# EBI-Metagenomics/deciphon-old

Measured on AMD Instinct MI355X. Metric: Gcell-updates/sec, higher is better.
Workload: dtype f32

## Files before the change

deciphon-old_amd/csrc/dcp_gpu.hip:

```cpp
#include "dcp_kernels.h"
#include "dcp_f64.h"

#include <hip/hip_runtime.h>

#include <algorithm>
#include <cmath>
#include <cstdarg>
#include <cstdio>
#include <cstring>
#include <limits>
#include <map>
#include <new>
#include <string>
#include <queue>
#include <vector>

namespace
{

struct SizeClass
{
    int R, W;
    unsigned cap() const { return 64u * (unsigned)R * (unsigned)W; }
};
// ... 1414 lines not shown
    {
        if (c->qorder_q0 != q_begin || c->qorder_q1 != q_end || c->qorder_nt != ql_nt)
        {
            unsigned const NTq = ql_nt, slots = NTq / 64u;
            std::vector<uint32_t> ord(nq);
            for (unsigned i = 0; i < nq; ++i)
                ord[i] = i;
            std::stable_sort(ord.begin(), ord.end(), [&](uint32_t x, uint32_t y) {
                return c->seq_len[q_begin + x] < c->seq_len[q_begin + y];
            });
            std::vector<unsigned> len_sorted(nq);
            for (unsigned i = 0; i < nq; ++i)
                len_sorted[i] = c->seq_len[q_begin + ord[i]];
            QlPlan const plan = plan_query_groups(len_sorted.data(), nq, slots);
            unsigned const nqb = plan.nqb;
            if ((uint64_t)plan.plane_rows * NTq * 4u > 0xffffffffull)
                return c->fail(DCP_ENOMEM, "sequences too long for the query-lane kernel (%u plane rows): use kernel = 1", plan.plane_rows);
            size_t const nslot_words = (size_t)nqb * slots + 1u, ngroup_words = plan.groups.size() * 4u;
            size_t const need_stage = (size_t)nq + nqb + 1u + nslot_words + ngroup_words;
            if (!c->ev_qstage) HIP_TRY(c, hipEventCreateWithFlags(&c->ev_qstage, hipEventDisableTiming));
            else HIP_TRY(c, hipEventSynchronize(c->ev_qstage));
            if (c->h_qstage_n < need_stage)
            {
                if (c->h_qstage) (void)hipHostFree(c->h_qstage);
                c->h_qstage = nullptr, c->h_qstage_n = 0;
                HIP_TRY(c, hipHostMalloc((void **)&c->h_qstage, need_stage * sizeof(uint32_t), hipHostMallocDefault));
                c->h_qstage_n = need_stage;
            }
            uint32_t *const h_ord = c->h_qstage, *const wt_off = h_ord + nq, *const h_slots = wt_off + nqb + 1u,
                           *const h_groups = h_slots + nslot_words;
            static_assert(sizeof(dcp_ql_group) == 4 * sizeof(uint32_t), "group records travel as four words");
// ... 85 lines not shown
                qa.redo_base[k] = (unsigned)tot;
                qa.redo_cap[k] = cap;
                tot += cap;
                uint64_t const tpb = dcp_rowsweep_tasks_per_block(kClasses[k].W);
                uint64_t g = std::min<uint64_t>((cap + tpb - 1) / tpb, 8ull * c->num_cus);
                redo_grid[k] = (unsigned)((g + 7) / 8 * 8);
            }
            if (c->d_redo.n < tot) HIP_TRY(c, c->d_redo.alloc((size_t)tot));
        }
        if (!c->d_redo_n.p) HIP_TRY(c, c->d_redo_n.alloc(DCP_MAX_CLASSES + 2));
        HIP_TRY(c, hipMemsetAsync(c->d_redo_n.p, 0, (DCP_MAX_CLASSES + 2) * sizeof(unsigned), c->stream));
        qa.redo = c->d_redo.p;
        qa.redo_n = c->d_redo_n.p;
        qa.redo_overflow = c->d_redo_n.p + DCP_MAX_CLASSES;
        qa.ring_error = c->d_redo_n.p + DCP_MAX_CLASSES + 1;
        uint64_t const per_block = (uint64_t)dcp_qlane_scratch_planes() * (uint64_t)qa.plane_rows * NT;
        uint64_t const budget = (uint64_t)64 << 28;
        uint64_t fit = per_block ? budget / per_block : 0;
        uint64_t const resident_blocks = (uint64_t)ql_blocks_per_cu * c->num_cus;
        unsigned nblocks = (unsigned)std::min<uint64_t>(std::min<uint64_t>(ntasks, resident_blocks), fit);
        if (use_w3) nblocks = (nblocks + 2u) / 3u * 3u;
        if (nblocks == 0)
            return c->fail(DCP_ENOMEM, "sequences too long for the query-lane kernel (%u plane rows): use kernel = 1", qa.plane_rows);
        size_t const need = (size_t)nblocks * per_block;
        if (c->d_scratch.n < need) HIP_TRY(c, c->d_scratch.alloc(need));
        qa.scratch = c->d_scratch.p;
        HIP_TRY(c, hipMemsetAsync(c->d_task_counter.p, 0, sizeof(unsigned), c->stream));
        HIP_TRY(c, hipEventRecord(c->ev_start, c->stream));
        if (two_stage ? dcp_launch_qlane2(&qa, nblocks, c->stream)
                      : use_w3 ? dcp_launch_qlane_w3(&qa, nblocks / 3u, c->stream)
                               : dcp_launch_qlane(&qa, nblocks, NT, c->stream))
// ... 611 lines not shown
```

deciphon-old_amd/csrc/dcp_kernels.h:

```cpp
#ifndef DCP_KERNELS_H
#define DCP_KERNELS_H

#include "dcp_host.h"
#include <stdint.h>

struct dcp_prof_meta
{
    uint64_t emis_off;
    uint32_t trans_off;
    uint32_t core_size;
    uint32_t ldk;
    uint32_t pidx;
    uint32_t flags;
    uint32_t width;
};
#define DCP_PROF_EXACT_E 1u

struct dcp_mp_group
{
    uint64_t emis_off;
    uint32_t trans_off;
    uint32_t ldk;
    uint32_t in_off;
    uint32_t nparts;
// ... 172 lines not shown
unsigned dcp_segsweep_blocks(unsigned nprof, unsigned nq);
int dcp_launch_rowsweep_grid(int R, int W, dcp_scan_args const *a, int stg, unsigned bw, void *stream,
                             unsigned pad_lds,
                             int prefetch2);
unsigned dcp_rowsweep_max_block_waves(int R, int W, int stg);
unsigned dcp_rowsweep_stage_bytes(int R, int stg);
int dcp_launch_qlane(dcp_qlane_args const *a, unsigned nblocks, unsigned nt, void *stream);
int dcp_launch_qlane2(dcp_qlane_args const *a, unsigned nblocks, void *stream);
unsigned dcp_qlane2_lds_bytes(void);
int dcp_launch_qlane_w3(dcp_qlane_args const *a, unsigned nblocks, void *stream);
int dcp_launch_qlane_transpose(dcp_qlane_args const *a, unsigned nt, void *stream);
void dcp_launch_trace(dcp_trace_args const *a, unsigned nhits, void *stream);
int dcp_launch_trace_forward(int R, int W, dcp_scan_args const *a, unsigned nblocks, void *stream);
unsigned dcp_qlane_block_size(void);
unsigned dcp_qlane_tile_nodes(void);
unsigned dcp_qlane_scratch_planes(void);
unsigned dcp_qlane_diag_build(void);
unsigned dcp_qlane_group_rows(unsigned lmax);
unsigned dcp_qlane_window_planes(void);
unsigned dcp_qlane_exact_e_by_redo(void);
#ifdef __cplusplus
}
#endif

#endif
```

deciphon-old_amd/csrc/dcp_qlane.hip:

```cpp
#include "dcp_kernels.h"

#include <hip/hip_runtime.h>
#include <type_traits>

namespace
{
constexpr int NC = DCP_NCODES;

#ifndef DCP_QLANE_RECOMPUTE_B
#define DCP_QLANE_RECOMPUTE_B 1
#endif
constexpr bool kRecomputeB = DCP_QLANE_RECOMPUTE_B != 0;
#ifndef DCP_QLANE_WD
#define DCP_QLANE_WD 5
#endif
constexpr unsigned kWD = DCP_QLANE_WD;
constexpr unsigned kPlanes = kRecomputeB ? 3u : 4u;
#ifndef DCP_QLANE_DIAG
#define DCP_QLANE_DIAG 0
#endif

#ifndef DCP_QL_WPLANE
#define DCP_QL_WPLANE 1
#endif
#ifndef DCP_QL_IN16
#define DCP_QL_IN16 1
#endif
#ifndef DCP_QL_EM
#define DCP_QL_EM 1
#endif
constexpr bool kWPlane = DCP_QL_WPLANE != 0, kIn16 = DCP_QL_IN16 != 0, kEM = DCP_QL_EM != 0;

// ... 88 lines not shown
        }
    }
}

__device__ __forceinline__ float ld_off(float const *base, unsigned boff)
{
    return *reinterpret_cast<float const *>(reinterpret_cast<char const *>(base) + boff);
}
typedef uint32_t const __attribute__((address_space(1))) *gu32_ptr;
typedef uint16_t const __attribute__((address_space(1))) *gu16_ptr;
typedef char const __attribute__((address_space(1))) *gchar_ptr;
__device__ __forceinline__ void st_off(float *base, unsigned boff, float v)
{
    *reinterpret_cast<float *>(reinterpret_cast<char *>(base) + boff) = v;
}

struct Ring
{
    float B[5], Xm[5], Xd[5], Em[5];
};

enum
{
    IO_HBM = 1,
    IO_LDS = 2
};
constexpr unsigned kRD = 16;
constexpr unsigned kRLanes = 256;
constexpr unsigned kRingPlaneBytes = kRD * kRLanes * 4u;
#ifndef DCP_Q2_SKEW
#define DCP_Q2_SKEW 4
#endif
#ifndef DCP_Q2_HYST
#define DCP_Q2_HYST 1
// ... 51 lines not shown
constexpr unsigned kRingSpinBound = 1u << 23;
constexpr unsigned kRingPoison = 0x7fffff00u;
__device__ __forceinline__ unsigned ring_wait(LdsLink const &lk, unsigned need)
{
    lds_uint *flag = (lds_uint *)(lk.base + lk.peer_flag);
    unsigned v = __builtin_amdgcn_readfirstlane(flag_load(flag));
#if DCP_Q2_BOUND
    unsigned spins = 0;
#pragma nounroll
    while (v < need)
    {
        __builtin_amdgcn_s_sleep(DCP_Q2_SLEEP);
        v = __builtin_amdgcn_readfirstlane(flag_load(flag));
        if (__builtin_expect(++spins == kRingSpinBound, 0))
        {
            typedef unsigned __attribute__((address_space(1))) *gerr_ptr;
            gerr_ptr const err = *(gerr_ptr __attribute__((address_space(3))) *)(lk.base + kL2Err);
            __hip_atomic_store(err, 1u, __ATOMIC_RELAXED, __HIP_MEMORY_SCOPE_AGENT);
            flag_store((lds_uint *)(lk.base + kL2Abort), 1u);
            flag_store(flag, kRingPoison);
            v = kRingPoison;
            __builtin_amdgcn_s_waitcnt(0x0070);
        }
    }
#else
    while (v < need)
    {
        __builtin_amdgcn_s_sleep(DCP_Q2_SLEEP);
        v = __builtin_amdgcn_readfirstlane(flag_load(flag));
    }
#endif
    DCP_ISA_MARK("DCP_RING_ACQUIRED");
    return v;
}
__device__ __forceinline__ float ring_ld(LdsLink const &lk, unsigned rowoff, unsigned plane)
{
    return *(lds_float *)(lk.base + ((rowoff & (kRingPlaneBytes - 1u)) | kL2Ring) + plane * kRingPlaneBytes);
}
__device__ __forceinline__ void ring_st(LdsLink const &lk, unsigned rowoff, unsigned plane, float v)
{
    *(lds_float *)(lk.base + ((rowoff & (kRingPlaneBytes - 1u)) | kL2Ring) + plane * kRingPlaneBytes) = v;
}
__device__ __forceinline__ void ring_publish(LdsLink const &lk, unsigned rowoff, unsigned row)
{
    flag_store((lds_uint *)(lk.base + lk.my_flag + (rowoff & (kRLanes * 4u - 1u))), row);
}

template <bool FIRST>
__device__ __forceinline__ void ring_fetch_x(Ring &r, int slot, float const *pXm, float const *pXd,
                                             float const *pEm, unsigned off)
{
    if constexpr (!FIRST)
    {
        r.Xm[slot] = ld_off(pXm, off);
        r.Xd[slot] = ld_off(pXd, off);
        r.Em[slot] = ld_off(pEm, off);
    }
}
template <bool FIRST>
__device__ __forceinline__ void ring_fetch_b(Ring &r, int slot, float const *pB, unsigned off)
{
    if constexpr (!kRecomputeB && !FIRST) r.B[slot] = ld_off(pB, off);
}
template <bool FIRST>
__device__ __forceinline__ void ring_fetch(Ring &r, int slot, float const *pB, float const *pXm,
                                           float const *pXd, float const *pEm, unsigned off)
{
    ring_fetch_x<FIRST>(r, slot, pXm, pXd, pEm, off);
    ring_fetch_b<FIRST>(r, slot, pB, off);
}

struct GatherOff
{
    unsigned a[5];
};
template <unsigned BASE> struct GatherMasks
{
    unsigned base, m[4];
    __device__ __forceinline__ GatherMasks()
    {
        static_assert((BASE & 0x3fffu) == 0u, "the base must not overlap the window's 14 bits");
        base = BASE;
        if constexpr (BASE != 0u) asm volatile("" : "+s"(base));
#pragma unroll
        for (int l = 0; l < 4; ++l)
// ... 31 lines not shown
            reinterpret_cast<char const *>(tabIN) + (IN16 ? g.a[l] + first[l] * 16u : (g.a[l] >> 1) + first[l] * 8u));
        in.eI[l] = v.x;
        in.eN[l] = v.y;
    }
}

template <int R> __device__ __forceinline__ float comp(float4 const &v)
{
    return R == 0 ? v.x : R == 1 ? v.y : R == 2 ? v.z : v.w;
}

template <int G, bool FIRST, bool LAST, int PH, int NT, int D, int IN = IO_HBM, int OUT = IO_HBM, unsigned TBASE = 0u,
          bool IN16 = kIn16>
__device__ __forceinline__ void ql_row(QState<G> &s, TileTrans<G> const &tr, float const *tabM,
                                       float2 const *tabIN, GatherOff &go,
                                       unsigned wn, RowIn &in, Ring &ring, float *pB, float *pXm,
                                       float *pXd, float *pEm, unsigned &off, LaneXt const &xt,
                                       bool live, bool at_end, bool &dirty, SweepOut &o,
                                       LdsLink const &lk, unsigned jrow, GatherMasks<TBASE> const &gm
#if DCP_QLANE_DIAG & 4
                                       , unsigned &off2, unsigned din
#endif
                                       )
{
    constexpr int KT = 4 * G;
    constexpr int s1 = (PH + 4) % 5, s2 = (PH + 3) % 5, s3 = (PH + 2) % 5, s4 = (PH + 1) % 5, s5 = PH;
    float const ni = ninf();

    static_assert(G <= 2, "gather_match<GROUP> is instantiated for groups 0 and 1");
    float4 e[G > 1 ? G - 1 : 1][5];
    if constexpr (G > 1)
    {
#pragma unroll
        for (int l = 0; l < 5; ++l)
            e[0][l] = gather_match<1>(tabM, go, l);
    }

    {
        constexpr int per_row = ((FIRST || IN != IO_HBM) ? 0 : 3) + ((LAST || OUT != IO_HBM) ? 0 : 3) +
                                ((!kRecomputeB && !FIRST) ? 1 : 0) + ((!kRecomputeB && FIRST) ? 1 : 0) + 1;
        constexpr int vm = ((D < (int)kWD ? D : (int)kWD) - 1) * per_row;
        constexpr int lgkm = G > 1 ? 5 : 0;
        __builtin_amdgcn_s_waitcnt((vm & 15) | ((vm >> 4) << 14) | (7 << 4) | (lgkm << 8));
    }
    __builtin_amdgcn_sched_barrier(0);
    float Xm = ni, Xd = ni, E = ni, Bj = ring.B[PH];
    if constexpr (!FIRST)
    {
        Xm = ring.Xm[PH];
        Xd = ring.Xd[PH];
        E = ring.Em[PH];
    }
    float eI[5], eN[5];
#pragma unroll
    for (int l = 0; l < 5; ++l)
    {
        eI[l] = in.eI[l];
        eN[l] = in.eN[l];
    }

    if constexpr (FIRST || kRecomputeB)
    {
        float const N = mx5(s.PN[s1] + eN[0], s.PN[s2] + eN[1], s.PN[s3] + eN[2],
                            s.PN[s4] + eN[3], s.PN[s5] + eN[4]);
        s.PN[PH] = N + xt.NN;
        Bj = N + xt.NB;
        if constexpr (FIRST)
        {
            float const Rn = mx5(s.PR[s1] + eN[0], s.PR[s2] + eN[1], s.PR[s3] + eN[2],
                                 s.PR[s4] + eN[3], s.PR[s5] + eN[4]);
            s.PR[PH] = Rn + xt.RR;
            o.Rn = at_end ? Rn : o.Rn;
            if constexpr (!kRecomputeB) st_off(pB, off, Bj);
        }
    }

    float pm = ni, pi = ni, pd = ni;
    float m_even = ni;
    auto node = [&](int k, float e0, float e1, float e2, float e3, float e4) {
        float const m = mx5(s.P[s1][k] + e0, s.P[s2][k] + e1, s.P[s3][k] + e2, s.P[s4][k] + e3,
                            s.P[s5][k] + e4);
        float const iv = mx5(s.Q[s1][k] + eI[0], s.Q[s2][k] + eI[1], s.Q[s3][k] + eI[2],
                             s.Q[s4][k] + eI[3], s.Q[s5][k] + eI[4]);
        float d, pin;
        if (k == 0)
        {
            d = Xd;
            pin = Xm;
// ... 11 lines not shown
        else E = mx3(E, m, d);
        s.P[PH][k] = fmaxf(Bj + tr.ent[k], pin);
        s.Q[PH][k] = fmaxf(m + tr.mi[k], iv + tr.ii[k]);
        pm = m, pi = iv, pd = d;
    };

    node(0, in.e0[0].x, in.e0[1].x, in.e0[2].x, in.e0[3].x, in.e0[4].x);
    node(1, in.e0[0].y, in.e0[1].y, in.e0[2].y, in.e0[3].y, in.e0[4].y);
    node(2, in.e0[0].z, in.e0[1].z, in.e0[2].z, in.e0[3].z, in.e0[4].z);
    node(3, in.e0[0].w, in.e0[1].w, in.e0[2].w, in.e0[3].w, in.e0[4].w);

    if constexpr (!FIRST && IN == IO_HBM)
    {
        asm volatile("" : "+v"(off) : "v"(E));
#if DCP_QLANE_DIAG & 4
        ring_fetch_x<FIRST>(ring, (PH + D) % 5, pXm + din, pXd + din, pEm + din, off);
#else
        ring_fetch_x<FIRST>(ring, (PH + D) % 5, pXm + D * NT, pXd + D * NT, pEm + D * NT, off);
#endif
    }

    __builtin_amdgcn_s_waitcnt(0xC07F | (0 << 8));
    go = gather_off<TBASE>(wn, gm);
    ql_fetch<G, FIRST, LAST, IN16>(in, tabM, tabIN, go);
    if constexpr (!FIRST && IN == IO_LDS)
    {
        constexpr int sl = (PH + 1) % 5;
        DCP_ISA_MARK("DCP_RING_TAKE");
        unsigned const nxt = off + kRLanes * 4u;
        ring.Xm[sl] = ring_ld(lk, nxt, 0);
        ring.Xd[sl] = ring_ld(lk, nxt, 1);
        ring.Em[sl] = ring_ld(lk, nxt, 2);
        DCP_ISA_MARK("DCP_RING_TAKEN");
        ring_publish(lk, off, jrow + 1u);
        DCP_ISA_MARK("DCP_RING_TAKE_END");
    }

#pragma unroll
    for (int g = 1; g < G; ++g)
    {
        float4 const *eg = e[g - 1];
        node(4 * g + 0, eg[0].x, eg[1].x, eg[2].x, eg[3].x, eg[4].x);
        node(4 * g + 1, eg[0].y, eg[1].y, eg[2].y, eg[3].y, eg[4].y);
        node(4 * g + 2, eg[0].z, eg[1].z, eg[2].z, eg[3].z, eg[4].z);
        node(4 * g + 3, eg[0].w, eg[1].w, eg[2].w, eg[3].w, eg[4].w);
    }

    if constexpr (!kRecomputeB && !FIRST)
    {
        asm volatile("" : "+v"(off) : "v"(pm));
        ring_fetch_b<FIRST>(ring, (PH + D) % 5, pB + D * NT, off);
    }

    if constexpr (!LAST)
    {
        float const oXm = mx3(pm + tr.mm[KT], pi + tr.im[KT], pd + tr.dm[KT]);
        float const oXd = fmaxf(pm + tr.md[KT], pd + tr.dd[KT]);
        if constexpr (OUT == IO_LDS)
        {
            DCP_ISA_MARK("DCP_RING_DATA");
            ring_st(lk, off, 0, oXm);
            ring_st(lk, off, 1, oXd);
            ring_st(lk, off, 2, E);
            DCP_ISA_MARK("DCP_RING_FLAG");
            ring_publish(lk, off, jrow);
            DCP_ISA_MARK("DCP_RING_DATA_END");
        }
        else
        {
#if DCP_QLANE_DIAG & 4
            unsigned const offw = off2;
#else
            unsigned const offw = off;
#endif
            st_off(pXm, offw, oXm);
            st_off(pXd, offw, oXd);
            st_off(pEm, offw, E);
        }
    }
    else
    {
        float const J = mx5(s.PJ[s1] + eN[0], s.PJ[s2] + eN[1], s.PJ[s3] + eN[2], s.PJ[s4] + eN[3],
                            s.PJ[s5] + eN[4]);
        float const C = mx5(s.PC[s1] + eN[0], s.PC[s2] + eN[1], s.PC[s3] + eN[2], s.PC[s4] + eN[3],
                            s.PC[s5] + eN[4]);
        float const B1 = fmaxf(E + xt.EB, J + xt.JB);
        dirty = dirty || (live && B1 > Bj);
        s.PJ[PH] = fmaxf(E + xt.EJ, J + xt.JJ);
        s.PC[PH] = fmaxf(E + xt.EC, C + xt.CC);
        o.E = at_end ? E : o.E;
        o.C = at_end ? C : o.C;
    }
}

template <int G, bool FIRST, bool LAST, int NT, int D, int IN = IO_HBM, int OUT = IO_HBM, unsigned TBASE = 0u,
          bool IN16 = kIn16>
__device__ __forceinline__ void ql_sweep(cfloat *tt, float const *tabM, float2 const *tabIN,
                                         uint32_t const *__restrict__ wordsT, unsigned rowbase,
                                         unsigned L, unsigned Lwave, bool active, float *sc,
                                         size_t plane, unsigned tid, LaneXt const &xt, bool &dirty,
                                         SweepOut &o, LdsLink lk
#if DCP_QLANE_DIAG & 4
                                         , unsigned tile_odd
#endif
                                         )
{
    constexpr int KT = 4 * G;
#if DCP_QLANE_DIAG & 4
    unsigned const rowstep = tile_odd ? 0u : (unsigned)NT;
    unsigned const rowstep_out = tile_odd ? (unsigned)NT : 0u;
    unsigned const din = (unsigned)D * rowstep;
    unsigned off2 = tid * 4u;
#else
    constexpr unsigned rowstep = (DCP_QLANE_DIAG & 2) ? 0u : (unsigned)NT;
#endif
// ... 5 lines not shown
    for (int h = 0; h < 5; ++h)
    {
#pragma unroll
        for (int k = 0; k < KT; ++k)
            s.P[h][k] = ni, s.Q[h][k] = ni;
        s.PN[h] = ni, s.PR[h] = ni, s.PJ[h] = ni, s.PC[h] = ni;
    }
    {
        float const B0 = 0.0f + xt.SB;
#pragma unroll
        for (int k = 0; k < KT; ++k)
            s.P[0][k] = B0 + tr.ent[k];
        s.PN[0] = 0.0f + xt.SN;
        s.PR[0] = 0.0f;
    }
    float *pXm = sc, *pXd = sc + plane, *pEm = sc + 2 * plane, *pB = sc + (kRecomputeB ? 0 : 3) * plane;
    unsigned off = (rowbase * (unsigned)NT + tid) * 4u;

    unsigned j = 1;
    static_assert(kWPlane, "the packed-word sequence planes are gone (round 4): a slot's groups are addressed by plane row");
    typedef uint16_t wq_t;
    wq_t wq[5];
    unsigned w;
    unsigned lane2 = tid * 2u;
    gu16_ptr const wpl = (gu16_ptr)wordsT + (size_t)rowbase * (unsigned)NT;
    asm volatile("" : "+v"(lane2));
    {
        w = wpl[NT + tid];
#pragma unroll
        for (int r = 2; r < 7; ++r)
            wq[r % 5] = wpl[r * NT + tid];
        __builtin_amdgcn_sched_barrier(0);
        __builtin_amdgcn_s_waitcnt(0x0F70);
    }
    RowIn in;
    Ring ring;
#pragma unroll
    for (int l = 0; l < 5; ++l)
    {
        in.e0[l] = float4{ni, ni, ni, ni}, in.eI[l] = ni, in.eN[l] = ni;
        ring.B[l] = ring.Xm[l] = ring.Xd[l] = ring.Em[l] = ni;
    }
    GatherMasks<TBASE> const gm;
    GatherOff go = gather_off<TBASE>(w, gm);
    ql_fetch<G, FIRST, LAST, IN16>(in, tabM, tabIN, go);
    if constexpr (!FIRST && IN == IO_LDS)
    {
        static_assert(NT == (int)kRLanes, "the ring's row stride is the scratch planes' row stride");
        unsigned const need0 = rowbase + (Lwave < kRingSkew ? Lwave : kRingSkew);
        lk.seen = ring_wait(lk, need0);
        DCP_ISA_MARK("DCP_RING_TAKE");
        ring.Xm[1] = ring_ld(lk, off, 0);
        ring.Xd[1] = ring_ld(lk, off, 1);
        ring.Em[1] = ring_ld(lk, off, 2);
        DCP_ISA_MARK("DCP_RING_TAKEN");
        ring_publish(lk, off, rowbase + 1u);
        DCP_ISA_MARK("DCP_RING_TAKE_END");
    }
    else
    {
        lk.seen = 0u;
#pragma unroll
        for (int r = 0; r < D; ++r)
            ring_fetch<(FIRST || IN != IO_HBM)>(ring, (r + 1) % 5, pB, pXm, pXd, pEm, off + (unsigned)r * rowstep * 4u);
    }

#if DCP_QLANE_DIAG & 8
#ifndef DCP_QLANE_DIAG_ROWS
#define DCP_QLANE_DIAG_ROWS 256u
#endif
#define QL_DIAG8_WRAP off &= (DCP_QLANE_DIAG_ROWS * (unsigned)NT * 4u - 1u);
#else
#define QL_DIAG8_WRAP
#endif
#if DCP_QLANE_DIAG & 4
#define QL_DIAG4_ARGS , off2, din
#define QL_DIAG4_STEP off2 += rowstep_out * 4u;
#else
#define QL_DIAG4_ARGS
#define QL_DIAG4_STEP
#endif
#define QL_ROW(PH)                                                                         \
    {                                                                                      \
                                                 \
        unsigned const pos = j + 1u;                                                       \
        ql_row<G, FIRST, LAST, PH, NT, D, IN, OUT, TBASE, IN16>(s, tr, tabM, tabIN, go,              \
                                   (unsigned)wq[(PH + 1) % 5], in, ring, pB, pXm,                    \
                                   pXd, pEm, off, xt, active && j <= L, active && j == L,  \
                                   dirty, o, lk, rowbase + j, gm QL_DIAG4_ARGS);           \
        {    \
             \
             \
             \
             \
            gu16_ptr wrow = wpl + (pos + 5u) * (unsigned)NT;                                     \
            asm volatile("" : "+s"(wrow));                                                   \
            asm volatile("" : "+v"(lane2));  \
            wq[(PH + 1) % 5] = *(gu16_ptr)((gchar_ptr)wrow + lane2);                          \
        }                                                                                    \
        off += rowstep * 4u;                                                                     \
        QL_DIAG8_WRAP                                                                            \
        QL_DIAG4_STEP                                                                            \
        ++j;                                                                               \
// ... 54 lines not shown
    g.rowbase = gd->rowbase;
    g.has = lane < nq;
    g.q = g.has ? a.qorder[qfirst + lane] : 0u;
    g.L = g.has ? a.seq_len[g.q] : 0u;
    g.Lwave = gd->lmax;
    float const *__restrict__ x = a.xtrans + (size_t)g.q * DCP_XSTRIDE;
    g.xt.RR = x[DCP_X_RR], g.xt.SB = x[DCP_X_SB], g.xt.SN = x[DCP_X_SN], g.xt.NN = x[DCP_X_NN];
    g.xt.NB = x[DCP_X_NB], g.xt.ET = x[DCP_X_ET], g.xt.EC = x[DCP_X_EC], g.xt.CC = x[DCP_X_CC];
    g.xt.CT = x[DCP_X_CT], g.xt.EB = x[DCP_X_EB], g.xt.EJ = x[DCP_X_EJ], g.xt.JJ = x[DCP_X_JJ];
    g.xt.JB = x[DCP_X_JB];
    __builtin_amdgcn_s_waitcnt(0x0F70);
    __builtin_amdgcn_sched_barrier(0);
}
__device__ __forceinline__ unsigned park_off(GroupLane const &g, unsigned NT, unsigned col)
{
    return ((g.rowbase + g.Lwave + 8u) * NT + col) * 4u;
}

__device__ __forceinline__ void ql_publish(dcp_qlane_args const &a, dcp_ql_prof const &pm, unsigned q, float nul, float alt,
                                           bool redo)
{
    if (redo)
    {
        unsigned const cls = pm.cls;
        unsigned const i = atomicAdd(a.redo_n + cls, 1u);
        if (i < a.redo_cap[cls]) a.redo[a.redo_base[cls] + i] = dcp_pair{q, pm.rs_slot};
        else *a.redo_overflow = 1u;
        return;
    }
    size_t const oi = (size_t)q * a.nprof_total + pm.pidx;
    if (a.out_null) a.out_null[oi] = nul;
// ... 6 lines not shown
    }
}

}

template <int G, int NT, int D, bool ROWS = false>
__global__ __launch_bounds__(NT, NT / 128) void viterbi_qlane_kernel(dcp_qlane_args a)
{
    constexpr int KT = 4 * G;
    constexpr int TAB_FLOATS = G * NC * 4;
    __shared__ __attribute__((aligned(16))) float lds[TAB_FLOATS + (kIn16 ? 4 : 2) * NC];
    __shared__ unsigned s_task;
    float *tabM = lds;
    float2 *tabIN = reinterpret_cast<float2 *>(lds + TAB_FLOATS);
    unsigned const tid = threadIdx.x;
    size_t const plane = (size_t)a.plane_rows * (unsigned)NT;
    float *const sc = a.scratch + (size_t)blockIdx.x * kPlanes * plane;
    constexpr unsigned SLOTS = (unsigned)NT / 64u;

    for (;;)
    {
        if (tid == 0) s_task = atomicAdd(a.task_counter, 1u);
        __syncthreads();
        unsigned const task = __builtin_amdgcn_readfirstlane(s_task);
        __syncthreads();
        if (task >= a.ntasks) break;
        unsigned const slot = a.nprof - 1u - task / a.nqblocks;
        unsigned const qb = task % a.nqblocks;
        dcp_ql_prof const pm = a.profs[slot];
        unsigned const T = pm.ntiles;
        unsigned const sidx = __builtin_amdgcn_readfirstlane(qb * SLOTS + (tid >> 6));
        cu32 *sf = (cu32 *)(unsigned long long)a.slot_first;
// ... 17 lines not shown
            cfloat *tt = as_const(a.ttrans + pm.ttrans_off + (size_t)t * (KT + 1) * 8);
            bool const first = t == 0, last = t + 1 == T;
            for (unsigned gi = g0; gi < g1; ++gi)
            {
                if (!(single && t_loaded)) load_group(a, gi, tid & 63u, g);
                t_loaded = true;
                if (g.Lwave == 0u) continue;
                SweepOut o{ninf(), ninf(), ninf()};
                bool dirty = false;
#if DCP_QLANE_DIAG & 4
#define QL_DIAG4_TILE , (t & 1u)
#else
#define QL_DIAG4_TILE
#endif
#define QL_SWEEP(F, L_)                                                                          \
    ql_sweep<G, F, L_, NT, D>(tt, tabM, tabIN, wordsT, g.rowbase, g.L, g.Lwave, g.has, sc, plane, tid, g.xt, dirty, o, LdsLink{} QL_DIAG4_TILE)
                if (first && last) QL_SWEEP(true, true);
                else if (first) QL_SWEEP(true, false);
                else if (last) QL_SWEEP(false, true);
                else QL_SWEEP(false, false);
#undef QL_SWEEP
                unsigned const po = park_off(g, (unsigned)NT, tid);
                if (first && !last) st_off(sc, po, o.Rn);
                if (last && g.has)
                {
                    float const nul = first ? o.Rn : ld_off(sc, po);
                    ql_publish(a, pm, g.q, nul, fmaxf(o.E + g.xt.ET, o.C + g.xt.CT), dirty || (kEM && pm.needs_exact_e));
                }
            }
        }
    }
// ... 3 lines not shown
__global__ __launch_bounds__(512, 2) void viterbi_qlane2_kernel(dcp_qlane_args a)
{
    constexpr int NT = (int)kRLanes;
    constexpr int KT = 4 * G;
    __shared__ __attribute__((aligned(16))) float lds[kL2Bytes / 4u];
    unsigned const wv = threadIdx.x >> 6;
#if DCP_Q2_STAGEMAP == 0
    unsigned const stage = __builtin_amdgcn_readfirstlane(wv & 1u);
    unsigned const tid = ((wv >> 1) << 6) | (threadIdx.x & 63u);
#else
    unsigned const stage = __builtin_amdgcn_readfirstlane(wv >> 2);
    unsigned const tid = threadIdx.x & 255u;
#endif
    unsigned *const s_task_p = reinterpret_cast<unsigned *>(lds + kL2Task / 4u);
    float *const tabM = lds + (stage ? kL2Tab1 / 4u : 0u);
    size_t const plane = (size_t)a.plane_rows * (unsigned)NT;
    float *const sc = a.scratch + (size_t)blockIdx.x * kPlanes * plane;
    constexpr unsigned SLOTS = (unsigned)NT / 64u;

#if DCP_Q2_PRIO == 1
    if (stage == 1u) __builtin_amdgcn_s_setprio(1);
#elif DCP_Q2_PRIO == 2
    if (stage == 0u) __builtin_amdgcn_s_setprio(1);
#endif
    LdsLink lk;
    lk.base = (lds_char *)lds;
    lk.my_flag = stage == 0u ? kL2FlagP : kL2FlagC;
    lk.peer_flag = (stage == 0u ? kL2FlagC : kL2FlagP) + (tid & ~63u) * 4u;
    lk.seen = 0u;
    if (threadIdx.x == 0) *(unsigned **)(lds + kL2Err / 4u) = a.ring_error;
    unsigned *const s_abort_p = reinterpret_cast<unsigned *>(lds + kL2Abort / 4u);

// ... 41 lines not shown
            if (!mine || (stalled && st == 0u) || __builtin_amdgcn_readfirstlane(*s_abort_p) != 0u) continue;
            cfloat *tt = as_const(a.ttrans + pm.ttrans_off + (size_t)t * (KT + 1) * 8);
            bool const first = t == 0u, last = t + 1u == T;
#if DCP_QLANE_DIAG & 4
#error "the two-stage kernel has no DIAG=4 build"
#endif
            for (unsigned gi = g0; gi < g1; ++gi)
            {
                if (!(single && t_loaded)) load_group(a, gi, tid & 63u, g);
                t_loaded = true;
                if (g.Lwave == 0u) continue;
                SweepOut o{ninf(), ninf(), ninf()};
                bool dirty = false;
#define QL2_SWEEP(F, L_, IN_, OUT_, TB_)                                                                  \
    ql_sweep<G, F, L_, NT, D, IN_, OUT_, TB_, false>(tt, lds, reinterpret_cast<float2 const *>(lds + (kL2TabIN - TB_ / 2u) / 4u), \
                                              wordsT, g.rowbase, g.L, g.Lwave, g.has, sc, plane, tid, g.xt, dirty, o, lk)
                if (stage == 0u)
                {
                    if (first && last) QL2_SWEEP(true, true, IO_HBM, IO_HBM, 0u);
                    else if (first) QL2_SWEEP(true, false, IO_HBM, IO_LDS, 0u);
                    else if (last) QL2_SWEEP(false, true, IO_HBM, IO_HBM, 0u);
                    else QL2_SWEEP(false, false, IO_HBM, IO_LDS, 0u);
                }
                else
                {
                    if (last) QL2_SWEEP(false, true, IO_LDS, IO_HBM, kL2Tab1);
                    else QL2_SWEEP(false, false, IO_LDS, IO_HBM, kL2Tab1);
                }
#undef QL2_SWEEP
                unsigned const po = park_off(g, (unsigned)NT, tid);
                if (first) st_off(sc, po, o.Rn);
                if (last)
                {
                    st_off(sc + plane, po, fmaxf(o.E + g.xt.ET, o.C + g.xt.CT));
                    st_off(sc + 2 * plane, po, dirty ? 1.0f : 0.0f);
                }
            }
        }
        __syncthreads();

        if (stage != final_stage) continue;
        for (unsigned gi = g0; gi < g1; ++gi)
        {
            cgroup *gd = (cgroup *)(unsigned long long)(a.groups + gi);
            GroupLane ge;
            ge.rowbase = gd->rowbase, ge.Lwave = gd->lmax;
            if (ge.Lwave == 0u || (tid & 63u) >= gd->nq) continue;
            unsigned const q = a.qorder[gd->qfirst + (tid & 63u)];
            unsigned const po = park_off(ge, (unsigned)NT, tid);
            float const nul = ld_off(sc, po), alt = ld_off(sc + plane, po);
            bool const dirty = ld_off(sc + 2 * plane, po) != 0.0f;
            ql_publish(a, pm, q, nul, alt, dirty || (kEM && pm.needs_exact_e));
        }
    }
}

template <int G, int D, bool ROWS = false>
__global__ __launch_bounds__(192, 1) void viterbi_qlane_w3_kernel(dcp_qlane_args a)
{
    constexpr int NT = 64;
    constexpr int KT = 4 * G;
    constexpr int TAB_FLOATS = G * NC * 4;
    constexpr int SLICE = TAB_FLOATS + 2 * NC;
    __shared__ __attribute__((aligned(16))) float lds[3 * SLICE];
    unsigned const wv = __builtin_amdgcn_readfirstlane(threadIdx.x >> 6);
    unsigned const tid = threadIdx.x & 63u;
    float *const tabM = lds + wv * SLICE;
    float2 *const tabIN = reinterpret_cast<float2 *>(tabM + TAB_FLOATS);
    size_t const plane = (size_t)a.plane_rows * (unsigned)NT;
    float *const sc = a.scratch + ((size_t)blockIdx.x * 3u + wv) * kPlanes * plane;

    for (;;)
    {
        unsigned t0 = 0;
        if (tid == 0) t0 = atomicAdd(a.task_counter, 1u);
        unsigned const task = __builtin_amdgcn_readfirstlane(t0);
        if (task >= a.ntasks) break;
        unsigned const slot = a.nprof - 1u - task / a.nqblocks;
        unsigned const qb = task % a.nqblocks;
        dcp_ql_prof const pm = a.profs[slot];
        unsigned const T = pm.ntiles;
        cu32 *sf = (cu32 *)(unsigned long long)a.slot_first;
        unsigned const g0 = sf[qb], g1 = sf[qb + 1u];
        uint32_t const *__restrict__ wordsT = a.words_t + __builtin_amdgcn_readfirstlane(a.wt_off[qb]);
        {
// ... 7 lines not shown
        bool t_loaded = false;
        for (unsigned t = 0; t < T; ++t)
        {
            stage_tile_image<G, ROWS>(tabM, a, pm, t, tid, (unsigned)NT);
            compiler_fence();
            cfloat *tt = as_const(a.ttrans + pm.ttrans_off + (size_t)t * (KT + 1) * 8);
            bool const first = t == 0, last = t + 1 == T;
            for (unsigned gi = g0; gi < g1; ++gi)
            {
                if (!(single && t_loaded)) load_group(a, gi, tid, g);
                t_loaded = true;
                if (g.Lwave == 0u) continue;
                SweepOut o{ninf(), ninf(), ninf()};
                bool dirty = false;
#define QLW_SWEEP(F, L_)                                                                                  \
    ql_sweep<G, F, L_, NT, D, IO_HBM, IO_HBM, 0u, false>(tt, tabM, tabIN, wordsT, g.rowbase, g.L, g.Lwave, g.has, sc, plane, tid, g.xt, dirty, o, LdsLink{})
                if (first && last) QLW_SWEEP(true, true);
                else if (first) QLW_SWEEP(true, false);
                else if (last) QLW_SWEEP(false, true);
                else QLW_SWEEP(false, false);
#undef QLW_SWEEP
                unsigned const po = park_off(g, (unsigned)NT, tid);
                if (first && !last) st_off(sc, po, o.Rn);
                if (last && g.has)
                {
                    float const nul = first ? o.Rn : ld_off(sc, po);
                    ql_publish(a, pm, g.q, nul, fmaxf(o.E + g.xt.ET, o.C + g.xt.CT), dirty || (kEM && pm.needs_exact_e));
                }
            }
            compiler_fence();
        }
// ... 38 lines not shown
template <int G, int NT, int D>
static void launch_ql(dcp_qlane_args const *a, unsigned nblocks, hipStream_t s)
{
    if (a->tiles_from_rows) hipLaunchKernelGGL((viterbi_qlane_kernel<G, NT, D, true>), dim3(nblocks), dim3(NT), 0, s, *a);
    else hipLaunchKernelGGL((viterbi_qlane_kernel<G, NT, D>), dim3(nblocks), dim3(NT), 0, s, *a);
}

#ifndef DCP_QLANE_NT
#define DCP_QLANE_NT 256
#endif
#ifndef DCP_QLANE_D
#define DCP_QLANE_D 3
#endif
extern "C" unsigned dcp_qlane_block_size(void) { return DCP_QLANE_NT; }
extern "C" unsigned dcp_qlane_tile_nodes(void) { return 8u; }
extern "C" unsigned dcp_qlane_scratch_planes(void) { return kPlanes; }
extern "C" unsigned dcp_qlane_diag_build(void) { return DCP_QLANE_DIAG; }
extern "C" unsigned dcp_qlane_group_rows(unsigned lmax) { return (lmax + 11u) & ~1u; }
extern "C" unsigned dcp_qlane_window_planes(void) { return kWPlane ? 1u : 0u; }
extern "C" unsigned dcp_qlane_exact_e_by_redo(void) { return kEM ? 1u : 0u; }

extern "C" int dcp_launch_qlane_transpose(dcp_qlane_args const *a, unsigned nt, void *stream)
{
    if (nt == 64) hipLaunchKernelGGL((transpose_words_kernel<64>), dim3(a->nqblocks), dim3(64), 0, (hipStream_t)stream, *a);
    else if (nt == DCP_QLANE_NT)
        hipLaunchKernelGGL((transpose_words_kernel<DCP_QLANE_NT>), dim3(a->nqblocks), dim3(DCP_QLANE_NT), 0, (hipStream_t)stream, *a);
    else return 1;
    return 0;
}

extern "C" unsigned dcp_qlane2_lds_bytes(void) { return kL2Bytes; }
// ... 24 lines not shown
```

Baseline: 1437.

## Interleave query-lane scratch planes into per-cell records with nontemporal vector access

Result: faster. 1452, median of 6 (+1.0%).

```diff
diff --git a/deciphon-old_amd/csrc/dcp_gpu.hip b/deciphon-old_amd/csrc/dcp_gpu.hip
--- a/deciphon-old_amd/csrc/dcp_gpu.hip
+++ b/deciphon-old_amd/csrc/dcp_gpu.hip
@@ -1452,7 +1452,7 @@
                 len_sorted[i] = c->seq_len[q_begin + ord[i]];
             QlPlan const plan = plan_query_groups(len_sorted.data(), nq, slots);
             unsigned const nqb = plan.nqb;
-            if ((uint64_t)plan.plane_rows * NTq * 4u > 0xffffffffull)
+            if ((uint64_t)(plan.plane_rows + 8u) * NTq * (4u * dcp_qlane_record_floats()) > 0xffffffffull)
                 return c->fail(DCP_ENOMEM, "sequences too long for the query-lane kernel (%u plane rows): use kernel = 1", plan.plane_rows);
             size_t const nslot_words = (size_t)nqb * slots + 1u, ngroup_words = plan.groups.size() * 4u;
             size_t const need_stage = (size_t)nq + nqb + 1u + nslot_words + ngroup_words;
@@ -1568,7 +1568,7 @@
         qa.redo_n = c->d_redo_n.p;
         qa.redo_overflow = c->d_redo_n.p + DCP_MAX_CLASSES;
         qa.ring_error = c->d_redo_n.p + DCP_MAX_CLASSES + 1;
-        uint64_t const per_block = (uint64_t)dcp_qlane_scratch_planes() * (uint64_t)qa.plane_rows * NT;
+        uint64_t const per_block = (uint64_t)dcp_qlane_record_floats() * (uint64_t)qa.plane_rows * NT;
         uint64_t const budget = (uint64_t)64 << 28;
         uint64_t fit = per_block ? budget / per_block : 0;
         uint64_t const resident_blocks = (uint64_t)ql_blocks_per_cu * c->num_cus;
diff --git a/deciphon-old_amd/csrc/dcp_kernels.h b/deciphon-old_amd/csrc/dcp_kernels.h
--- a/deciphon-old_amd/csrc/dcp_kernels.h
+++ b/deciphon-old_amd/csrc/dcp_kernels.h
@@ -210,7 +210,7 @@
 int dcp_launch_trace_forward(int R, int W, dcp_scan_args const *a, unsigned nblocks, void *stream);
 unsigned dcp_qlane_block_size(void);
 unsigned dcp_qlane_tile_nodes(void);
-unsigned dcp_qlane_scratch_planes(void);
+unsigned dcp_qlane_record_floats(void);
 unsigned dcp_qlane_diag_build(void);
 unsigned dcp_qlane_group_rows(unsigned lmax);
 unsigned dcp_qlane_window_planes(void);
diff --git a/deciphon-old_amd/csrc/dcp_qlane.hip b/deciphon-old_amd/csrc/dcp_qlane.hip
--- a/deciphon-old_amd/csrc/dcp_qlane.hip
+++ b/deciphon-old_amd/csrc/dcp_qlane.hip
@@ -11,11 +11,16 @@
 #define DCP_QLANE_RECOMPUTE_B 1
 #endif
 constexpr bool kRecomputeB = DCP_QLANE_RECOMPUTE_B != 0;
+#ifndef DCP_QLANE_STREAM
+#define DCP_QLANE_STREAM 3
+#endif
+constexpr bool kStreamSt = (DCP_QLANE_STREAM & 1) != 0, kStreamLd = (DCP_QLANE_STREAM & 2) != 0;
 #ifndef DCP_QLANE_WD
 #define DCP_QLANE_WD 5
 #endif
 constexpr unsigned kWD = DCP_QLANE_WD;
-constexpr unsigned kPlanes = kRecomputeB ? 3u : 4u;
+typedef float f4v __attribute__((ext_vector_type(4)));
+constexpr unsigned kRecFloats = kRecomputeB ? 3u : 4u;
 #ifndef DCP_QLANE_DIAG
 #define DCP_QLANE_DIAG 0
 #endif
@@ -134,10 +139,42 @@
 {
     *reinterpret_cast<float *>(reinterpret_cast<char *>(base) + boff) = v;
 }
+typedef float f3v __attribute__((ext_vector_type(3), aligned(4)));
+template <bool WITH_B> __device__ __forceinline__ f4v ld_rec(float const *base, unsigned boff)
+{
+    char const *p = reinterpret_cast<char const *>(base) + boff;
+    if constexpr (WITH_B)
+    {
+        if constexpr (kStreamLd) return __builtin_nontemporal_load(reinterpret_cast<f4v const *>(p));
+        else return *reinterpret_cast<f4v const *>(p);
+    }
+    else
+    {
+        f3v v;
+        if constexpr (kStreamLd) v = __builtin_nontemporal_load(reinterpret_cast<f3v const *>(p));
+        else v = *reinterpret_cast<f3v const *>(p);
+        return f4v{v.x, v.y, v.z, 0.0f};
+    }
+}
+__device__ __forceinline__ void st_rec(float *base, unsigned boff, f4v v)
+{
+    char *const p = reinterpret_cast<char *>(base) + boff;
+    if constexpr (kRecFloats == 4u)
+    {
+        if constexpr (kStreamSt) __builtin_nontemporal_store(v, reinterpret_cast<f4v *>(p));
+        else *reinterpret_cast<f4v *>(p) = v;
+    }
+    else
+    {
+        f3v const w = v.xyz;
+        if constexpr (kStreamSt) __builtin_nontemporal_store(w, reinterpret_cast<f3v *>(p));
+        else *reinterpret_cast<f3v *>(p) = w;
+    }
+}
 
 struct Ring
 {
-    float B[5], Xm[5], Xd[5], Em[5];
+    f4v X[5];
 };
 
 enum
@@ -219,6 +256,7 @@
         v = __builtin_amdgcn_readfirstlane(flag_load(flag));
         if (__builtin_expect(++spins == kRingSpinBound, 0))
         {
+            DCP_ISA_MARK("DCP_RING_BOUND");
             typedef unsigned __attribute__((address_space(1))) *gerr_ptr;
             gerr_ptr const err = *(gerr_ptr __attribute__((address_space(3))) *)(lk.base + kL2Err);
             __hip_atomic_store(err, 1u, __ATOMIC_RELAXED, __HIP_MEMORY_SCOPE_AGENT);
@@ -226,6 +264,7 @@
             flag_store(flag, kRingPoison);
             v = kRingPoison;
             __builtin_amdgcn_s_waitcnt(0x0070);
+            DCP_ISA_MARK("DCP_RING_BOUND_END");
         }
     }
 #else
@@ -251,29 +290,12 @@
     flag_store((lds_uint *)(lk.base + lk.my_flag + (rowoff & (kRLanes * 4u - 1u))), row);
 }
 
-template <bool FIRST>
-__device__ __forceinline__ void ring_fetch_x(Ring &r, int slot, float const *pXm, float const *pXd,
-                                             float const *pEm, unsigned off)
-{
-    if constexpr (!FIRST)
-    {
-        r.Xm[slot] = ld_off(pXm, off);
-        r.Xd[slot] = ld_off(pXd, off);
-        r.Em[slot] = ld_off(pEm, off);
-    }
-}
-template <bool FIRST>
-__device__ __forceinline__ void ring_fetch_b(Ring &r, int slot, float const *pB, unsigned off)
-{
-    if constexpr (!kRecomputeB && !FIRST) r.B[slot] = ld_off(pB, off);
-}
-template <bool FIRST>
-__device__ __forceinline__ void ring_fetch(Ring &r, int slot, float const *pB, float const *pXm,
-                                           float const *pXd, float const *pEm, unsigned off)
-{
-    ring_fetch_x<FIRST>(r, slot, pXm, pXd, pEm, off);
-    ring_fetch_b<FIRST>(r, slot, pB, off);
-}
+template <bool FIRST, bool WITH_B>
+__device__ __forceinline__ void ring_fetch_x(Ring &r, int slot, float const *sc, unsigned roff)
+{
+    if constexpr (!FIRST) r.X[slot] = ld_rec<WITH_B>(sc, roff);
+}
+__device__ __forceinline__ unsigned rec_off(unsigned off) { return off * kRecFloats; }
 
 struct GatherOff
 {
@@ -335,8 +357,8 @@
           bool IN16 = kIn16>
 __device__ __forceinline__ void ql_row(QState<G> &s, TileTrans<G> const &tr, float const *tabM,
                                        float2 const *tabIN, GatherOff &go,
-                                       unsigned wn, RowIn &in, Ring &ring, float *pB, float *pXm,
-                                       float *pXd, float *pEm, unsigned &off, LaneXt const &xt,
+                                       unsigned wn, RowIn &in, Ring &ring, float *sc,
+                                       unsigned &off, LaneXt const &xt,
                                        bool live, bool at_end, bool &dirty, SweepOut &o,
                                        LdsLink const &lk, unsigned jrow, GatherMasks<TBASE> const &gm
 #if DCP_QLANE_DIAG & 4
@@ -345,6 +367,7 @@
                                        )
 {
     constexpr int KT = 4 * G;
+    constexpr bool BREC = !kRecomputeB && !FIRST && IN == IO_HBM;
     constexpr int s1 = (PH + 4) % 5, s2 = (PH + 3) % 5, s3 = (PH + 2) % 5, s4 = (PH + 1) % 5, s5 = PH;
     float const ni = ninf();
 
@@ -358,19 +381,20 @@
     }
 
     {
-        constexpr int per_row = ((FIRST || IN != IO_HBM) ? 0 : 3) + ((LAST || OUT != IO_HBM) ? 0 : 3) +
-                                ((!kRecomputeB && !FIRST) ? 1 : 0) + ((!kRecomputeB && FIRST) ? 1 : 0) + 1;
+        constexpr int per_row = ((FIRST || IN != IO_HBM) ? 0 : 1) + ((LAST || OUT != IO_HBM) ? 0 : 1) + 1;
         constexpr int vm = ((D < (int)kWD ? D : (int)kWD) - 1) * per_row;
         constexpr int lgkm = G > 1 ? 5 : 0;
         __builtin_amdgcn_s_waitcnt((vm & 15) | ((vm >> 4) << 14) | (7 << 4) | (lgkm << 8));
     }
     __builtin_amdgcn_sched_barrier(0);
-    float Xm = ni, Xd = ni, E = ni, Bj = ring.B[PH];
+    float Xm = ni, Xd = ni, E = ni, Bj = ni;
     if constexpr (!FIRST)
     {
-        Xm = ring.Xm[PH];
-        Xd = ring.Xd[PH];
-        E = ring.Em[PH];
+        f4v const x = ring.X[PH];
+        Xm = x.x;
+        Xd = x.y;
+        E = x.z;
+        if constexpr (BREC) Bj = x.w;
     }
     float eI[5], eN[5];
 #pragma unroll
@@ -380,7 +404,7 @@
         eN[l] = in.eN[l];
     }
 
-    if constexpr (FIRST || kRecomputeB)
+    if constexpr (!BREC)
     {
         float const N = mx5(s.PN[s1] + eN[0], s.PN[s2] + eN[1], s.PN[s3] + eN[2],
                             s.PN[s4] + eN[3], s.PN[s5] + eN[4]);
@@ -392,7 +416,6 @@
                                  s.PR[s4] + eN[3], s.PR[s5] + eN[4]);
             s.PR[PH] = Rn + xt.RR;
             o.Rn = at_end ? Rn : o.Rn;
-            if constexpr (!kRecomputeB) st_off(pB, off, Bj);
         }
     }
 
@@ -434,9 +457,9 @@
     {
         asm volatile("" : "+v"(off) : "v"(E));
 #if DCP_QLANE_DIAG & 4
-        ring_fetch_x<FIRST>(ring, (PH + D) % 5, pXm + din, pXd + din, pEm + din, off);
+        ring_fetch_x<FIRST, BREC>(ring, (PH + D) % 5, sc + din * kRecFloats, rec_off(off));
 #else
-        ring_fetch_x<FIRST>(ring, (PH + D) % 5, pXm + D * NT, pXd + D * NT, pEm + D * NT, off);
+        ring_fetch_x<FIRST, BREC>(ring, (PH + D) % 5, sc + D * NT * kRecFloats, rec_off(off));
 #endif
     }
 
@@ -448,9 +471,9 @@
         constexpr int sl = (PH + 1) % 5;
         DCP_ISA_MARK("DCP_RING_TAKE");
         unsigned const nxt = off + kRLanes * 4u;
-        ring.Xm[sl] = ring_ld(lk, nxt, 0);
-        ring.Xd[sl] = ring_ld(lk, nxt, 1);
-        ring.Em[sl] = ring_ld(lk, nxt, 2);
+        ring.X[sl].x = ring_ld(lk, nxt, 0);
+        ring.X[sl].y = ring_ld(lk, nxt, 1);
+        ring.X[sl].z = ring_ld(lk, nxt, 2);
         DCP_ISA_MARK("DCP_RING_TAKEN");
         ring_publish(lk, off, jrow + 1u);
         DCP_ISA_MARK("DCP_RING_TAKE_END");
@@ -464,12 +487,6 @@
         node(4 * g + 1, eg[0].y, eg[1].y, eg[2].y, eg[3].y, eg[4].y);
         node(4 * g + 2, eg[0].z, eg[1].z, eg[2].z, eg[3].z, eg[4].z);
         node(4 * g + 3, eg[0].w, eg[1].w, eg[2].w, eg[3].w, eg[4].w);
-    }
-
-    if constexpr (!kRecomputeB && !FIRST)
-    {
-        asm volatile("" : "+v"(off) : "v"(pm));
-        ring_fetch_b<FIRST>(ring, (PH + D) % 5, pB + D * NT, off);
     }
 
     if constexpr (!LAST)
@@ -493,9 +510,7 @@
 #else
             unsigned const offw = off;
 #endif
-            st_off(pXm, offw, oXm);
-            st_off(pXd, offw, oXd);
-            st_off(pEm, offw, E);
+            st_rec(sc, rec_off(offw), f4v{oXm, oXd, E, Bj});
         }
     }
     else
@@ -518,7 +533,7 @@
 __device__ __forceinline__ void ql_sweep(cfloat *tt, float const *tabM, float2 const *tabIN,
                                          uint32_t const *__restrict__ wordsT, unsigned rowbase,
                                          unsigned L, unsigned Lwave, bool active, float *sc,
-                                         size_t plane, unsigned tid, LaneXt const &xt, bool &dirty,
+                                         unsigned tid, LaneXt const &xt, bool &dirty,
                                          SweepOut &o, LdsLink lk
 #if DCP_QLANE_DIAG & 4
                                          , unsigned tile_odd
@@ -554,7 +569,6 @@
         s.PN[0] = 0.0f + xt.SN;
         s.PR[0] = 0.0f;
     }
-    float *pXm = sc, *pXd = sc + plane, *pEm = sc + 2 * plane, *pB = sc + (kRecomputeB ? 0 : 3) * plane;
     unsigned off = (rowbase * (unsigned)NT + tid) * 4u;
 
     unsigned j = 1;
@@ -579,7 +593,7 @@
     for (int l = 0; l < 5; ++l)
     {
         in.e0[l] = float4{ni, ni, ni, ni}, in.eI[l] = ni, in.eN[l] = ni;
-        ring.B[l] = ring.Xm[l] = ring.Xd[l] = ring.Em[l] = ni;
+        ring.X[l] = f4v{ni, ni, ni, ni};
     }
     GatherMasks<TBASE> const gm;
     GatherOff go = gather_off<TBASE>(w, gm);
@@ -590,9 +604,9 @@
         unsigned const need0 = rowbase + (Lwave < kRingSkew ? Lwave : kRingSkew);
         lk.seen = ring_wait(lk, need0);
         DCP_ISA_MARK("DCP_RING_TAKE");
-        ring.Xm[1] = ring_ld(lk, off, 0);
-        ring.Xd[1] = ring_ld(lk, off, 1);
-        ring.Em[1] = ring_ld(lk, off, 2);
+        ring.X[1].x = ring_ld(lk, off, 0);
+        ring.X[1].y = ring_ld(lk, off, 1);
+        ring.X[1].z = ring_ld(lk, off, 2);
         DCP_ISA_MARK("DCP_RING_TAKEN");
         ring_publish(lk, off, rowbase + 1u);
         DCP_ISA_MARK("DCP_RING_TAKE_END");
@@ -602,7 +616,7 @@
         lk.seen = 0u;
 #pragma unroll
         for (int r = 0; r < D; ++r)
-            ring_fetch<(FIRST || IN != IO_HBM)>(ring, (r + 1) % 5, pB, pXm, pXd, pEm, off + (unsigned)r * rowstep * 4u);
+            ring_fetch_x<(FIRST || IN != IO_HBM), (!kRecomputeB && !FIRST && IN == IO_HBM)>(ring, (r + 1) % 5, sc, rec_off(off + (unsigned)r * rowstep * 4u));
     }
 
 #if DCP_QLANE_DIAG & 8
@@ -625,8 +639,8 @@
                                                  \
         unsigned const pos = j + 1u;                                                       \
         ql_row<G, FIRST, LAST, PH, NT, D, IN, OUT, TBASE, IN16>(s, tr, tabM, tabIN, go,              \
-                                   (unsigned)wq[(PH + 1) % 5], in, ring, pB, pXm,                    \
-                                   pXd, pEm, off, xt, active && j <= L, active && j == L,  \
+                                   (unsigned)wq[(PH + 1) % 5], in, ring, sc,                         \
+                                   off, xt, active && j <= L, active && j == L,            \
                                    dirty, o, lk, rowbase + j, gm QL_DIAG4_ARGS);           \
         {    \
              \
@@ -711,7 +725,7 @@
 }
 __device__ __forceinline__ unsigned park_off(GroupLane const &g, unsigned NT, unsigned col)
 {
-    return ((g.rowbase + g.Lwave + 8u) * NT + col) * 4u;
+    return ((g.rowbase + g.Lwave + 8u) * NT + col) * (kRecFloats * 4u);
 }
 
 __device__ __forceinline__ void ql_publish(dcp_qlane_args const &a, dcp_ql_prof const &pm, unsigned q, float nul, float alt,
@@ -748,8 +762,7 @@
     float *tabM = lds;
     float2 *tabIN = reinterpret_cast<float2 *>(lds + TAB_FLOATS);
     unsigned const tid = threadIdx.x;
-    size_t const plane = (size_t)a.plane_rows * (unsigned)NT;
-    float *const sc = a.scratch + (size_t)blockIdx.x * kPlanes * plane;
+    float *const sc = a.scratch + (size_t)blockIdx.x * kRecFloats * a.plane_rows * (unsigned)NT;
     constexpr unsigned SLOTS = (unsigned)NT / 64u;
 
     for (;;)
@@ -797,7 +810,7 @@
 #define QL_DIAG4_TILE
 #endif
 #define QL_SWEEP(F, L_)                                                                          \
-    ql_sweep<G, F, L_, NT, D>(tt, tabM, tabIN, wordsT, g.rowbase, g.L, g.Lwave, g.has, sc, plane, tid, g.xt, dirty, o, LdsLink{} QL_DIAG4_TILE)
+    ql_sweep<G, F, L_, NT, D>(tt, tabM, tabIN, wordsT, g.rowbase, g.L, g.Lwave, g.has, sc, tid, g.xt, dirty, o, LdsLink{} QL_DIAG4_TILE)
                 if (first && last) QL_SWEEP(true, true);
                 else if (first) QL_SWEEP(true, false);
                 else if (last) QL_SWEEP(false, true);
@@ -831,8 +844,7 @@
 #endif
     unsigned *const s_task_p = reinterpret_cast<unsigned *>(lds + kL2Task / 4u);
     float *const tabM = lds + (stage ? kL2Tab1 / 4u : 0u);
-    size_t const plane = (size_t)a.plane_rows * (unsigned)NT;
-    float *const sc = a.scratch + (size_t)blockIdx.x * kPlanes * plane;
+    float *const sc = a.scratch + (size_t)blockIdx.x * kRecFloats * a.plane_rows * (unsigned)NT;
     constexpr unsigned SLOTS = (unsigned)NT / 64u;
 
 #if DCP_Q2_PRIO == 1
@@ -904,7 +916,7 @@
                 bool dirty = false;
 #define QL2_SWEEP(F, L_, IN_, OUT_, TB_)                                                                  \
     ql_sweep<G, F, L_, NT, D, IN_, OUT_, TB_, false>(tt, lds, reinterpret_cast<float2 const *>(lds + (kL2TabIN - TB_ / 2u) / 4u), \
-                                              wordsT, g.rowbase, g.L, g.Lwave, g.has, sc, plane, tid, g.xt, dirty, o, lk)
+                                              wordsT, g.rowbase, g.L, g.Lwave, g.has, sc, tid, g.xt, dirty, o, lk)
                 if (stage == 0u)
                 {
                     if (first && last) QL2_SWEEP(true, true, IO_HBM, IO_HBM, 0u);
@@ -922,8 +934,8 @@
                 if (first) st_off(sc, po, o.Rn);
                 if (last)
                 {
-                    st_off(sc + plane, po, fmaxf(o.E + g.xt.ET, o.C + g.xt.CT));
-                    st_off(sc + 2 * plane, po, dirty ? 1.0f : 0.0f);
+                    st_off(sc, po + 4u, fmaxf(o.E + g.xt.ET, o.C + g.xt.CT));
+                    st_off(sc, po + 8u, dirty ? 1.0f : 0.0f);
                 }
             }
         }
@@ -938,9 +950,8 @@
             if (ge.Lwave == 0u || (tid & 63u) >= gd->nq) continue;
             unsigned const q = a.qorder[gd->qfirst + (tid & 63u)];
             unsigned const po = park_off(ge, (unsigned)NT, tid);
-            float const nul = ld_off(sc, po), alt = ld_off(sc + plane, po);
-            bool const dirty = ld_off(sc + 2 * plane, po) != 0.0f;
-            ql_publish(a, pm, q, nul, alt, dirty || (kEM && pm.needs_exact_e));
+            f3v const pk = *reinterpret_cast<f3v const *>(reinterpret_cast<char const *>(sc) + po);
+            ql_publish(a, pm, q, pk.x, pk.y, pk.z != 0.0f || (kEM && pm.needs_exact_e));
         }
     }
 }
@@ -957,8 +968,7 @@
     unsigned const tid = threadIdx.x & 63u;
     float *const tabM = lds + wv * SLICE;
     float2 *const tabIN = reinterpret_cast<float2 *>(tabM + TAB_FLOATS);
-    size_t const plane = (size_t)a.plane_rows * (unsigned)NT;
-    float *const sc = a.scratch + ((size_t)blockIdx.x * 3u + wv) * kPlanes * plane;
+    float *const sc = a.scratch + ((size_t)blockIdx.x * 3u + wv) * kRecFloats * a.plane_rows * (unsigned)NT;
 
     for (;;)
     {
@@ -996,7 +1006,7 @@
                 SweepOut o{ninf(), ninf(), ninf()};
                 bool dirty = false;
 #define QLW_SWEEP(F, L_)                                                                                  \
-    ql_sweep<G, F, L_, NT, D, IO_HBM, IO_HBM, 0u, false>(tt, tabM, tabIN, wordsT, g.rowbase, g.L, g.Lwave, g.has, sc, plane, tid, g.xt, dirty, o, LdsLink{})
+    ql_sweep<G, F, L_, NT, D, IO_HBM, IO_HBM, 0u, false>(tt, tabM, tabIN, wordsT, g.rowbase, g.L, g.Lwave, g.has, sc, tid, g.xt, dirty, o, LdsLink{})
                 if (first && last) QLW_SWEEP(true, true);
                 else if (first) QLW_SWEEP(true, false);
                 else if (last) QLW_SWEEP(false, true);
@@ -1065,7 +1075,7 @@
 #endif
 extern "C" unsigned dcp_qlane_block_size(void) { return DCP_QLANE_NT; }
 extern "C" unsigned dcp_qlane_tile_nodes(void) { return 8u; }
-extern "C" unsigned dcp_qlane_scratch_planes(void) { return kPlanes; }
+extern "C" unsigned dcp_qlane_record_floats(void) { return kRecFloats; }
 extern "C" unsigned dcp_qlane_diag_build(void) { return DCP_QLANE_DIAG; }
 extern "C" unsigned dcp_qlane_group_rows(unsigned lmax) { return (lmax + 11u) & ~1u; }
 extern "C" unsigned dcp_qlane_window_planes(void) { return kWPlane ? 1u : 0u; }
```
